# yl4579/StyleTTS2

Hardware: AMD Instinct MI355X
Metric: audio-seconds/sec (RTF^-1) end-to-end, 10 s utterance batch (higher is better)
Workload: dtype f32 (convs/linears: f16 hi/lo split, 3 MFMA products, fp32 accumulate)

## Files before the change

styletts2_amd/csrc/st2_misc.hip:

```cpp
#include "st2_common.h"

namespace {

__global__ __launch_bounds__(256) void conv1d_direct_kernel(const float* __restrict__ x, int64_t x_bs, int x_cs,
                                                            const float* __restrict__ w,
                                                            const float* __restrict__ bias, float* __restrict__ y,
                                                            int64_t y_bs, int y_cs, int C_in, int L_in_max, int L_out,
                                                            int ks, int stride, int pad, const int32_t* __restrict__ x_len,
                                                            const int32_t* __restrict__ y_len) {
  const int l = blockIdx.x * 256 + threadIdx.x;
  const int co = blockIdx.y;
  const int b = blockIdx.z;
  if (l >= L_out) return;
  const int L_in = x_len ? min(x_len[b], L_in_max) : L_in_max;
  if (y_len && l >= y_len[b]) {
    y[(int64_t)b * y_bs + (int64_t)co * y_cs + l] = 0.f;
    return;
  }
  const float* xb = x + (int64_t)b * x_bs;
  const float* wc = w + (int64_t)co * C_in * ks;
  float acc = 0.f;
  const int base = l * stride - pad;
  for (int ci = 0; ci < C_in; ++ci) {
    const float* xr = xb + (int64_t)ci * x_cs;
    for (int t = 0; t < ks; ++t) {
      const int p = base + t;
      if (p >= 0 && p < L_in) acc = fmaf(wc[ci * ks + t], xr[p], acc);
    }
  }
  if (bias) acc += bias[co];
  y[(int64_t)b * y_bs + (int64_t)co * y_cs + l] = acc;
}

__global__ __launch_bounds__(256) void phase_split_kernel(const float* __restrict__ x, int64_t x_bs, int x_cs, int L_in,
                                                          float* __restrict__ xp, int64_t p_bs, int p_cs, int Lu,
                                                          int stride, int pad) {
  const int pp = blockIdx.x * 256 + threadIdx.x;
  const int ci = blockIdx.y;
  const int b = blockIdx.z;
  if (pp >= Lu * stride) return;
  const int u = pp / stride;
  const int r = pp - u * stride;
  const int p = pp - pad;
  const float v = (p >= 0 && p < L_in) ? x[(int64_t)b * x_bs + (int64_t)ci * x_cs + p] : 0.f;
  xp[(int64_t)b * p_bs + (int64_t)(ci * stride + r) * p_cs + u] = v;
}

constexpr int CVT_TILE = 1024;
template <int S>
__global__ __launch_bounds__(256) void convt_interleave_kernel(const float* __restrict__ ph, int64_t p_bs, int p_cs,
                                                               const float* __restrict__ bias,
                                                               const float* __restrict__ add, int64_t a_bs, int a_cs,
                                                               float* __restrict__ out, int64_t o_bs, int o_cs, int C,
                                                               int stride_rt, int pad, int L_raw_max, int reflect_left,
                                                               float* __restrict__ part, int part_nt, int Lq_max,
                                                               const int32_t* __restrict__ q_len,
                                                               const int32_t* __restrict__ out_len) {
  extern __shared__ float cvt_tile[];
  __shared__ float red[2][4];
  const int stride = S ? S : stride_rt;
  const int co = blockIdx.y;
  const int b = blockIdx.z;
  const int L_out = out_len ? min(out_len[b], L_raw_max + reflect_left) : L_raw_max + reflect_left;
  const int Lq = q_len ? min(q_len[b], Lq_max) : Lq_max;
  const int o0 = blockIdx.x * CVT_TILE;
  if (o0 >= L_out) return;
  const int nq = CVT_TILE / stride + 3;
  const int nqp = nq | 1;
  const int l_lo = max(o0 - reflect_left, 0);
  const int q_lo = (l_lo + pad) / stride;
  {
    const float* pb = ph + (int64_t)b * p_bs + (int64_t)co * p_cs;
    const int total = stride * nq;
    constexpr int SB = 8;
    for (int e0 = threadIdx.x; e0 < total; e0 += 256 * SB) {
      float t[SB];
#pragma unroll
      for (int u = 0; u < SB; ++u) {
        const int e = min(e0 + u * 256, total - 1);
        const int r = e / nq, i = e - r * nq;
        t[u] = pb[(int64_t)r * C * p_cs + max(min(q_lo + i, Lq - 1), 0)];
      }
#pragma unroll
      for (int u = 0; u < SB; ++u) {
        const int e = e0 + u * 256;
        if (e < total) {
          const int r = e / nq, i = e - r * nq;
          cvt_tile[r * nqp + i] = (q_lo + i) < Lq ? t[u] : 0.f;
        }
      }
    }
  }
  __syncthreads();
  const float bj = bias ? bias[co] : 0.f;
  const float* ab = add ? add + (int64_t)b * a_bs + (int64_t)co * a_cs : nullptr;
  float* ob = out + (int64_t)b * o_bs + (int64_t)co * o_cs;
  auto staged_at = [&](int o) __attribute__((always_inline)) -> float {
    int l = o;
    if (reflect_left) l = (o == 0) ? 1 : o - 1;
    const int lp = l + pad;
    const int q = lp / stride;
    const int r = lp - q * stride;
    return cvt_tile[r * nqp + (q - q_lo)] + bj;
  };
  float shift = staged_at(o0);
  if (ab) shift += ab[o0];
  float s1 = 0.f, s2 = 0.f;
  const int o = o0 + 4 * threadIdx.x;
  if (o < L_out) {
    typedef float f4 __attribute__((ext_vector_type(4)));
    const bool full = o + 3 < L_out;
    const bool vec = full && ((reinterpret_cast<uintptr_t>(ob + o) & 15) == 0) && (!ab || (reinterpret_cast<uintptr_t>(ab + o) & 15) == 0);
    float v[4];
#pragma unroll
    for (int e = 0; e < 4; ++e) v[e] = (full || o + e < L_out) ? staged_at(o + e) : 0.f;
    if (ab) {
      if (vec) {
        const f4 a4 = *reinterpret_cast<const f4*>(ab + o);
#pragma unroll
        for (int e = 0; e < 4; ++e) v[e] += a4[e];
      } else {
#pragma unroll
        for (int e = 0; e < 4; ++e)
          if (full || o + e < L_out) v[e] += ab[o + e];
      }
    }
    if (vec) {
      *reinterpret_cast<f4*>(ob + o) = f4{v[0], v[1], v[2], v[3]};
    } else {
#pragma unroll
      for (int e = 0; e < 4; ++e)
        if (full || o + e < L_out) ob[o + e] = v[e];
    }
#pragma unroll
    for (int e = 0; e < 4; ++e)
      if (full || o + e < L_out) {
        const float dv = v[e] - shift;
        s1 += dv;
        s2 += dv * dv;
      }
  }
  if (part) {
    s1 = st2_wave_sum(s1);
    s2 = st2_wave_sum(s2);
    const int lane = threadIdx.x & 63, wave = threadIdx.x >> 6;
    if (lane == 0) {
      red[0][wave] = s1;
      red[1][wave] = s2;
    }
    __syncthreads();
    if (threadIdx.x == 0) {
      const float t1 = ((red[0][0] + red[0][1]) + red[0][2]) + red[0][3];
      const float t2 = ((red[1][0] + red[1][1]) + red[1][2]) + red[1][3];
      const int64_t slot = ((int64_t)b * C + co) * part_nt + blockIdx.x;
      reinterpret_cast<float2*>(part)[slot] = make_float2(t1, t2);
      part[(int64_t)gridDim.z * C * part_nt * 2 + slot] = shift;
    }
  }
}

__global__ __launch_bounds__(256) void adain_leaky_pool_kernel(const float* __restrict__ x, int64_t x_bs, int x_cs,
                                                               const float* __restrict__ stats,
                                                               const float* __restrict__ gamma,
                                                               const float* __restrict__ beta, int64_t gb_bs,
                                                               float slope, const float* __restrict__ w,
                                                               const float* __restrict__ bias, float* __restrict__ y,
                                                               int64_t y_bs, int y_cs, int C, int L_max,
                                                               const int32_t* __restrict__ len) {
  const int lo = blockIdx.x * 256 + threadIdx.x;
  const int c = blockIdx.y;
  const int b = blockIdx.z;
  const int L = len ? min(len[b], L_max) : L_max;
  if (lo >= 2 * L) return;
  const float mean = stats[((int64_t)b * C + c) * 2 + 0];
  const float rstd = stats[((int64_t)b * C + c) * 2 + 1];
  const float g = 1.0f + gamma[(int64_t)b * gb_bs + c];
  const float be = beta[(int64_t)b * gb_bs + c];
  const float* xr = x + (int64_t)b * x_bs + (int64_t)c * x_cs;
  auto act = [&](int i) -> float {
    float u = (xr[i] - mean) * rstd;
    u = g * u + be;
    return u >= 0.f ? u : u * slope;
  };
  const int j = lo >> 1;
  float v;
  if ((lo & 1) == 0) {
    v = act(j) * w[c * 3 + 1];
  } else {
    v = act(j) * w[c * 3 + 2];
    if (j + 1 < L) v += act(j + 1) * w[c * 3 + 0];
  }
  if (bias) v += bias[c];
  y[(int64_t)b * y_bs + (int64_t)c * y_cs + lo] = v;
}

__global__ __launch_bounds__(256) void add_chanvec_kernel(const float* __restrict__ x, int64_t x_bs, int x_cs,
                                                          const float* __restrict__ v, int64_t v_bs,
                                                          float* __restrict__ y, int64_t y_bs, int y_cs, int C,
                                                          int N) {
  const int n = blockIdx.x * 256 + threadIdx.x;
  const int c = blockIdx.y;
  const int b = blockIdx.z;
  if (n >= N) return;
  y[(int64_t)b * y_bs + (int64_t)c * y_cs + n] =
      x[(int64_t)b * x_bs + (int64_t)c * x_cs + n] + v[(int64_t)b * v_bs + c];
}

__global__ __launch_bounds__(64) void mean_tokens_kernel(const float* __restrict__ x, int64_t x_bs, int x_cs,
                                                         float* __restrict__ m, int64_t m_bs, int C, int N,
                                                         const int* __restrict__ len) {
  const int c = blockIdx.x;
  const int b = blockIdx.y;
  const float* xr = x + (int64_t)b * x_bs + (int64_t)c * x_cs;
  const int n_b = len ? min(max(len[b], 1), N) : N;
  double s = 0.0;
  for (int n = threadIdx.x; n < n_b; n += 64) s += (double)xr[n];
  s = st2_wave_sum(s);
  if (threadIdx.x == 0) m[(int64_t)b * m_bs + c] = (float)(s / (double)n_b);
}

__global__ __launch_bounds__(256) void axpbypcz_kernel(const float* __restrict__ x, float a,
                                                       const float* __restrict__ y, float b,
                                                       const float* __restrict__ z, float c, float* __restrict__ out,
                                                       int64_t n) {
  const int64_t i = (int64_t)blockIdx.x * 256 + threadIdx.x;
  if (i >= n) return;
  float v = a * x[i];
  if (y) v += b * y[i];
  if (z) v += c * z[i];
  out[i] = v;
}

}

extern "C" int st2_conv1d_direct(const float* x, int64_t x_bs, int32_t x_cs, const float* w, const float* bias,
                                 float* y, int64_t y_bs, int32_t y_cs, int32_t B, int32_t C_in, int32_t C_out,
                                 int32_t L_in, int32_t L_out, int32_t ks, int32_t stride, int32_t pad,
                                 void* stream) {
  return st2_conv1d_direct_len(x, x_bs, x_cs, w, bias, y, y_bs, y_cs, B, C_in, C_out, L_in, L_out, ks, stride, pad, nullptr,
                               nullptr, stream);
}

extern "C" int st2_conv1d_direct_len(const float* x, int64_t x_bs, int32_t x_cs, const float* w, const float* bias,
                                     float* y, int64_t y_bs, int32_t y_cs, int32_t B, int32_t C_in, int32_t C_out,
                                     int32_t L_in, int32_t L_out, int32_t ks, int32_t stride, int32_t pad,
                                     const int32_t* x_len, const int32_t* y_len, void* stream) {
  ST2_REQUIRE(x && w && y && B > 0 && C_in > 0 && C_out > 0 && L_in > 0 && L_out > 0 && ks > 0 && stride > 0,
              "st2_conv1d_direct: bad arguments");
  ST2_REQUIRE(C_out <= 65535 && B <= 65535, "st2_conv1d_direct: grid too large");
  hipStream_t s = reinterpret_cast<hipStream_t>(stream);
  hipLaunchKernelGGL(conv1d_direct_kernel, dim3(st2_cdiv(L_out, 256), C_out, B), dim3(256), 0, s, x, x_bs, x_cs, w,
                     bias, y, y_bs, y_cs, C_in, L_in, L_out, ks, stride, pad, x_len, y_len);
  ST2_CHECK_LAUNCH("st2_conv1d_direct");
  return 0;
}

extern "C" int st2_phase_split(const float* x, int64_t x_bs, int32_t x_cs, int32_t B, int32_t C, int32_t L_in,
                               int32_t stride, int32_t pad, float* xp, int64_t p_bs, int32_t p_cs, int32_t Lu,
                               void* stream) {
  ST2_REQUIRE(x && xp && B > 0 && C > 0 && L_in > 0 && stride > 0 && pad >= 0 && Lu > 0,
              "st2_phase_split: bad arguments");
  ST2_REQUIRE(C <= 65535 && B <= 65535 && (int64_t)Lu * stride < (int64_t)1 << 31, "st2_phase_split: grid too large");
  hipStream_t s = reinterpret_cast<hipStream_t>(stream);
  hipLaunchKernelGGL(phase_split_kernel, dim3(st2_cdiv((int64_t)Lu * stride, 256), C, B), dim3(256), 0, s, x, x_bs,
                     x_cs, L_in, xp, p_bs, p_cs, Lu, stride, pad);
  ST2_CHECK_LAUNCH("st2_phase_split");
  return 0;
}

extern "C" int st2_convt_interleave(const float* phases, int64_t p_bs, int32_t p_cs, int32_t Lq, const float* bias,
                                    const float* add, int64_t a_bs, int32_t a_cs, float* out, int64_t o_bs,
                                    int32_t o_cs, int32_t B, int32_t C, int32_t stride, int32_t pad, int32_t L_raw,
                                    int32_t reflect_left, void* stream) {
  return st2_convt_interleave_stats(phases, p_bs, p_cs, Lq, bias, add, a_bs, a_cs, out, o_bs, o_cs, B, C, stride, pad,
                                    L_raw, reflect_left, nullptr, 0, stream);
}

extern "C" int st2_convt_interleave_stats(const float* phases, int64_t p_bs, int32_t p_cs, int32_t Lq,
                                          const float* bias, const float* add, int64_t a_bs, int32_t a_cs, float* out,
                                          int64_t o_bs, int32_t o_cs, int32_t B, int32_t C, int32_t stride, int32_t pad,
                                          int32_t L_raw, int32_t reflect_left, float* part, int32_t part_nt,
                                          void* stream) {
  return st2_convt_interleave_stats_len(phases, p_bs, p_cs, Lq, bias, add, a_bs, a_cs, out, o_bs, o_cs, B, C, stride, pad, L_raw,
                                        reflect_left, part, part_nt, nullptr, nullptr, stream);
}

extern "C" int st2_convt_interleave_stats_len(const float* phases, int64_t p_bs, int32_t p_cs, int32_t Lq,
                                              const float* bias, const float* add, int64_t a_bs, int32_t a_cs, float* out,
                                              int64_t o_bs, int32_t o_cs, int32_t B, int32_t C, int32_t stride, int32_t pad,
                                              int32_t L_raw, int32_t reflect_left, float* part, int32_t part_nt,
                                              const int32_t* q_len, const int32_t* out_len, void* stream) {
  ST2_REQUIRE(!q_len == !out_len, "st2_convt_interleave_stats_len: q_len and out_len go together");
  ST2_REQUIRE(phases && out && B > 0 && C > 0 && stride > 0 && L_raw > 0 && Lq > 0,
              "st2_convt_interleave: bad arguments");
  ST2_REQUIRE(reflect_left == 0 || (reflect_left == 1 && L_raw >= 2), "st2_convt_interleave: bad reflect_left");
  ST2_REQUIRE(stride <= 64, "st2_convt_interleave: stride %d too large", stride);
  const int L_out = L_raw + reflect_left;
  const int nt = st2_cdiv(L_out, CVT_TILE);
  if (part) ST2_REQUIRE(part_nt >= nt && (reinterpret_cast<uintptr_t>(part) & 7) == 0,
                        "st2_convt_interleave: part_nt=%d < %d tiles (or part not 8-byte aligned)", part_nt, nt);
  ST2_REQUIRE(B <= 65535 && C <= 65535, "st2_convt_interleave: grid too large");
  hipStream_t s = reinterpret_cast<hipStream_t>(stream);
  const int nq = CVT_TILE / stride + 3;
  const size_t smem = (size_t)stride * (nq | 1) * sizeof(float);
#define ST2_CVT_LAUNCH(SV)                                                                                              \
  hipLaunchKernelGGL((convt_interleave_kernel<SV>), dim3(nt, C, B), dim3(256), smem, s, phases, p_bs, p_cs, bias, add, \
                     a_bs, a_cs, out, o_bs, o_cs, C, stride, pad, L_raw, reflect_left, part, part_nt, Lq, q_len, out_len)
  switch (stride) {
    case 2: ST2_CVT_LAUNCH(2); break;
    case 3: ST2_CVT_LAUNCH(3); break;
    case 5: ST2_CVT_LAUNCH(5); break;
    case 6: ST2_CVT_LAUNCH(6); break;
    case 10: ST2_CVT_LAUNCH(10); break;
    default: ST2_CVT_LAUNCH(0); break;
  }
#undef ST2_CVT_LAUNCH
  ST2_CHECK_LAUNCH("st2_convt_interleave");
  return 0;
}

extern "C" int st2_adain_leaky_pool(const float* x, int64_t x_bs, int32_t x_cs, const float* stats,
                                    const float* gamma, const float* beta, int64_t gb_bs, float slope, const float* w,
                                    const float* bias, float* y, int64_t y_bs, int32_t y_cs, int32_t B, int32_t C,
                                    int32_t L, void* stream) {
  return st2_adain_leaky_pool_len(x, x_bs, x_cs, stats, gamma, beta, gb_bs, slope, w, bias, y, y_bs, y_cs, B, C, L, nullptr,
                                  stream);
}

extern "C" int st2_adain_leaky_pool_len(const float* x, int64_t x_bs, int32_t x_cs, const float* stats,
                                        const float* gamma, const float* beta, int64_t gb_bs, float slope, const float* w,
                                        const float* bias, float* y, int64_t y_bs, int32_t y_cs, int32_t B, int32_t C,
                                        int32_t L, const int32_t* len, void* stream) {
  ST2_REQUIRE(x && stats && gamma && beta && w && y && B > 0 && C > 0 && L > 0,
              "st2_adain_leaky_pool: bad arguments");
  hipStream_t s = reinterpret_cast<hipStream_t>(stream);
  hipLaunchKernelGGL(adain_leaky_pool_kernel, dim3(st2_cdiv(2 * L, 256), C, B), dim3(256), 0, s, x, x_bs, x_cs,
                     stats, gamma, beta, gb_bs, slope, w, bias, y, y_bs, y_cs, C, L, len);
  ST2_CHECK_LAUNCH("st2_adain_leaky_pool");
  return 0;
}

extern "C" int st2_add_chanvec(const float* x, int64_t x_bs, int32_t x_cs, const float* v, int64_t v_bs, float* y,
                               int64_t y_bs, int32_t y_cs, int32_t B, int32_t C, int32_t N, void* stream) {
  ST2_REQUIRE(x && v && y && B > 0 && C > 0 && N > 0, "st2_add_chanvec: bad arguments");
  hipStream_t s = reinterpret_cast<hipStream_t>(stream);
  hipLaunchKernelGGL(add_chanvec_kernel, dim3(st2_cdiv(N, 256), C, B), dim3(256), 0, s, x, x_bs, x_cs, v, v_bs, y,
                     y_bs, y_cs, C, N);
  ST2_CHECK_LAUNCH("st2_add_chanvec");
  return 0;
}

extern "C" int st2_mean_tokens(const float* x, int64_t x_bs, int32_t x_cs, float* m, int64_t m_bs, int32_t B,
                               int32_t C, int32_t N, void* stream) {
  ST2_REQUIRE(x && m && B > 0 && C > 0 && N > 0, "st2_mean_tokens: bad arguments");
  hipStream_t s = reinterpret_cast<hipStream_t>(stream);
  hipLaunchKernelGGL(mean_tokens_kernel, dim3(C, B), dim3(64), 0, s, x, x_bs, x_cs, m, m_bs, C, N,
                     static_cast<const int*>(nullptr));
  ST2_CHECK_LAUNCH("st2_mean_tokens");
  return 0;
}

extern "C" int st2_mean_tokens_len(const float* x, int64_t x_bs, int32_t x_cs, float* m, int64_t m_bs, int32_t B,
                                   int32_t C, int32_t N, const int32_t* len, void* stream) {
  ST2_REQUIRE(x && m && B > 0 && C > 0 && N > 0, "st2_mean_tokens_len: bad arguments");
  hipStream_t s = reinterpret_cast<hipStream_t>(stream);
  hipLaunchKernelGGL(mean_tokens_kernel, dim3(C, B), dim3(64), 0, s, x, x_bs, x_cs, m, m_bs, C, N,
                     reinterpret_cast<const int*>(len));
  ST2_CHECK_LAUNCH("st2_mean_tokens_len");
  return 0;
}

extern "C" int st2_axpbypcz(const float* x, float a, const float* y, float b, const float* z, float c, float* out,
                            int64_t n, void* stream) {
  ST2_REQUIRE(x && out && n > 0, "st2_axpbypcz: bad arguments");
  hipStream_t s = reinterpret_cast<hipStream_t>(stream);
  hipLaunchKernelGGL(axpbypcz_kernel, dim3(st2_cdiv(n, 256)), dim3(256), 0, s, x, a, y, b, z, c, out, n);
  ST2_CHECK_LAUNCH("st2_axpbypcz");
  return 0;
}
```

styletts2_amd/csrc/st2_source.hip:

```cpp
#include "st2_common.h"

namespace {

__device__ __forceinline__ float torch_remainder1(float x) {
  float m = fmodf(x, 1.0f);
  if (m != 0.0f && m < 0.0f) m += 1.0f;
  return m;
}

__global__ __launch_bounds__(64) void sinegen_phase_kernel(const float* __restrict__ f0, int B, int F_max, int U, int H,
                                                           float sample_rate, float* __restrict__ phase_f,
                                                           const int32_t* __restrict__ f_len) {
  const int row = blockIdx.x;
  const int lane = threadIdx.x;
  const int b = row / H;
  const int h = row % H;
  const float mult = (float)(h + 1);
  const int F = f_len ? min(f_len[b], F_max) : F_max;
  const float* f = f0 + (int64_t)b * F_max;
  float* out = phase_f + ((int64_t)b * H + h) * F_max;
  const float two_pi_part = 3.14159274101257324219f;
  const float fu = (float)U;
  const int chunk = (F + 63) / 64;
  const int k0 = min(lane * chunk, F), k1 = min(k0 + chunk, F);
  double part = 0.0;
  for (int k = k0; k < k1; ++k) {
    const float fn = f[k] * mult;
    part += (double)torch_remainder1(fn / sample_rate);
  }
  double incl = part;
#pragma unroll
  for (int d = 1; d < 64; d <<= 1) {
    const double up = __shfl_up(incl, d, 64);
    if (lane >= d) incl += up;
  }
  double acc = __shfl_up(incl, 1, 64);
  if (lane == 0) acc = 0.0;
  for (int k = k0; k < k1; ++k) {
    const float fn = f[k] * mult;
    acc += (double)torch_remainder1(fn / sample_rate);
    const float c = (float)acc;
    out[k] = ((c * 2.0f) * two_pi_part) * fu;
  }
}

__global__ __launch_bounds__(256) void har_source_kernel(const float* __restrict__ f0, int F_max, int U, int H,
                                                         const float* __restrict__ noise,
                                                         const float* __restrict__ lin_w,
                                                         const float* __restrict__ lin_b, float sine_amp,
                                                         float noise_std, float voiced_threshold,
                                                         const float* __restrict__ phase_f,
                                                         float* __restrict__ out, const int32_t* __restrict__ f_len) {
  const int L_max = F_max * U;
  const int t = blockIdx.x * 256 + threadIdx.x;
  const int b = blockIdx.y;
  if (t >= L_max) return;
  const int F = f_len ? min(f_len[b], F_max) : F_max;
  const int L = F * U;
  if (t >= L) {
    out[(int64_t)b * L_max + t] = 0.f;
    return;
  }
  const float rs = (float)(1.0 / (double)U);
  float src = fmaf(rs, (float)t + 0.5f, -0.5f);
  src = src < 0.f ? 0.f : src;
  const int i0 = (int)src;
  const int i1 = min(i0 + 1, F - 1);
  const float w1 = src - (float)i0;
  const float w0 = 1.0f - w1;

  const float f0v = f0[(int64_t)b * F_max + t / U];
  const float uv = f0v > voiced_threshold ? 1.0f : 0.0f;
  const float noise_amp = uv * noise_std + ((1.0f - uv) * sine_amp) / 3.0f;

  const float* nz = noise + ((int64_t)b * L_max + t) * H;
  float acc = 0.f;
  for (int h = 0; h < H; ++h) {
    const float* pf = phase_f + ((int64_t)b * H + h) * F_max;
    const float ph = fmaf(w0, pf[i0], w1 * pf[i1]);
    const float sine = sinf(ph) * sine_amp;
    const float sw = sine * uv + noise_amp * nz[h];
    acc = fmaf(lin_w[h], sw, acc);
  }
  out[(int64_t)b * L_max + t] = tanhf(acc + lin_b[0]);
}

constexpr int MAXN = 32;
__global__ __launch_bounds__(256) void stft_kernel(const float* __restrict__ x, int L_max, int N, int hop,
                                                   float* __restrict__ har, int64_t har_bs, int har_cs,
                                                   const int32_t* __restrict__ len) {
  __shared__ float tw_c[MAXN], tw_s[MAXN], win[MAXN];
  if (threadIdx.x < N) {
    const double a = 2.0 * (double)threadIdx.x / (double)N;
    tw_c[threadIdx.x] = (float)cospi(a);
    tw_s[threadIdx.x] = (float)sinpi(a);
    win[threadIdx.x] = (float)(0.5 - 0.5 * cospi(a));
  }
  __syncthreads();
  const int m = blockIdx.x * 256 + threadIdx.x;
  const int b = blockIdx.y;
  if (m >= L_max / hop + 1) return;
  const int L = len ? min(max(len[b], N / 2 + 1), L_max) : L_max;
  const int M = L / hop + 1;
  const int NB = N / 2 + 1;
  float* hb = har + (int64_t)b * har_bs + m;
  if (m >= M) {
    for (int k = 0; k < 2 * NB; ++k) hb[(int64_t)k * har_cs] = 0.f;
    return;
  }
  const float* xb = x + (int64_t)b * L_max;
  float fr[MAXN];
  const int pad = N / 2;
#pragma unroll
  for (int n = 0; n < MAXN; ++n) {
    if (n < N) {
      int i = m * hop + n - pad;
      if (i < 0) i = -i;
      if (i >= L) i = 2 * (L - 1) - i;
      fr[n] = xb[i] * win[n];
    } else {
      fr[n] = 0.f;
    }
  }
  for (int k = 0; k < NB; ++k) {
    float re = 0.f, im = 0.f;
    int idx = 0;
#pragma unroll
    for (int n = 0; n < MAXN; ++n) {
      if (n < N) {
        re = fmaf(fr[n], tw_c[idx], re);
        im = fmaf(-fr[n], tw_s[idx], im);
        idx += k;
        if (idx >= N) idx -= N;
      }
    }
    hb[(int64_t)k * har_cs] = sqrtf(re * re + im * im);
    hb[(int64_t)(NB + k) * har_cs] = atan2f(im, re);
  }
}

__global__ __launch_bounds__(256) void istft_kernel(const float* __restrict__ sp, int64_t sp_bs, int sp_cs, int M_max,
                                                    int N, int hop, float* __restrict__ wave, int64_t wave_bs, int FRP,
                                                    const int32_t* __restrict__ m_len) {
  __shared__ float tw_c[MAXN], tw_s[MAXN], win[MAXN];
  extern __shared__ float ri[];
  if (threadIdx.x < N) {
    const double a = 2.0 * (double)threadIdx.x / (double)N;
    tw_c[threadIdx.x] = (float)cospi(a);
    tw_s[threadIdx.x] = (float)sinpi(a);
    win[threadIdx.x] = (float)(0.5 - 0.5 * cospi(a));
  }
  const int t = blockIdx.x * 256 + threadIdx.x;
  const int b = blockIdx.y;
  const int M = m_len ? min(max(m_len[b], 2), M_max) : M_max;
  const int Lw = hop * (M - 1);
  const int NB = N / 2 + 1;
  const float* sb = sp + (int64_t)b * sp_bs;
  {
    const int t0 = blockIdx.x * 256;
    const int tp0 = t0 + N / 2, tp1 = min(t0 + 255, Lw - 1) + N / 2;
    const int m_base = (tp0 - N + 1 <= 0) ? 0 : (tp0 - N + hop) / hop;
    const int m_last = min(tp1 / hop, M - 1);
    const int FR = m_last - m_base + 1;
    float* re_s = ri;
    float* im_s = ri + NB * FRP;
    for (int e = threadIdx.x; e < NB * FR; e += 256) {
      const int k = e / FR, f = e - k * FR;
      const float mag = sb[(int64_t)k * sp_cs + m_base + f];
      const float ph = sb[(int64_t)(NB + k) * sp_cs + m_base + f];
      re_s[k * FRP + f] = mag * cosf(ph);
      im_s[k * FRP + f] = mag * sinf(ph);
    }
  }
  __syncthreads();
  if (t >= Lw) {
    if (t < hop * (M_max - 1)) wave[(int64_t)b * wave_bs + t] = 0.f;
    return;
  }
  const int tp = t + N / 2;
  const int tp0 = (int)blockIdx.x * 256 + N / 2;
  const int m_base = (tp0 - N + 1 <= 0) ? 0 : (tp0 - N + hop) / hop;
  const float* re_s = ri;
  const float* im_s = ri + NB * FRP;
  int m_hi = tp / hop;
  if (m_hi > M - 1) m_hi = M - 1;
  int m_lo = (tp - N + hop) / hop;
  if (tp - N + 1 <= 0) m_lo = 0;
  const float inv_n = 1.0f / (float)N;
  float y = 0.f, env = 0.f;
  for (int m = m_lo; m <= m_hi; ++m) {
    const int n = tp - m * hop;
    float acc = 0.f;
    int idx = 0;
    const int f = m - m_base;
    for (int k = 0; k < NB; ++k) {
      const float re = re_s[k * FRP + f];
      const float im = im_s[k * FRP + f];
      if (k == 0 || k == N / 2) {
        acc += re * tw_c[idx];
      } else {
        acc += 2.0f * (re * tw_c[idx] - im * tw_s[idx]);
      }
      idx += n;
      if (idx >= N) idx -= N;
    }
    const float w = win[n];
    y += (acc * inv_n) * w;
    env += w * w;
  }
  wave[(int64_t)b * wave_bs + t] = y / env;
}

}

extern "C" int st2_har_source(const float* f0, int32_t B, int32_t F, int32_t U, int32_t H, const float* noise,
                              const float* lin_w, const float* lin_b, float sine_amp, float noise_std,
                              float voiced_threshold, float sample_rate, float* phase_scratch, float* out,
                              void* stream) {
  return st2_har_source_len(f0, B, F, U, H, noise, lin_w, lin_b, sine_amp, noise_std, voiced_threshold, sample_rate,
                            phase_scratch, out, nullptr, stream);
}

extern "C" int st2_har_source_len(const float* f0, int32_t B, int32_t F, int32_t U, int32_t H, const float* noise,
                                  const float* lin_w, const float* lin_b, float sine_amp, float noise_std,
                                  float voiced_threshold, float sample_rate, float* phase_scratch, float* out,
                                  const int32_t* f_len, void* stream) {
  ST2_REQUIRE(f0 && noise && lin_w && lin_b && phase_scratch && out, "st2_har_source: null pointer");
  ST2_REQUIRE(B > 0 && F > 0 && U > 0 && H > 0 && H <= 64, "st2_har_source: bad geometry");
  ST2_REQUIRE((int64_t)F * U < (1LL << 31), "st2_har_source: utterance too long");
  hipStream_t s = reinterpret_cast<hipStream_t>(stream);
  hipLaunchKernelGGL(sinegen_phase_kernel, dim3(B * H), dim3(64), 0, s, f0, B, F, U, H, sample_rate,
                     phase_scratch, f_len);
  ST2_CHECK_LAUNCH("st2_har_source(phase)");
  hipLaunchKernelGGL(har_source_kernel, dim3(st2_cdiv((int64_t)F * U, 256), B), dim3(256), 0, s, f0, F, U, H, noise,
                     lin_w, lin_b, sine_amp, noise_std, voiced_threshold, phase_scratch, out, f_len);
  ST2_CHECK_LAUNCH("st2_har_source");
  return 0;
}

extern "C" int st2_stft_mag_phase(const float* x, int32_t B, int32_t L, int32_t n_fft, int32_t hop, float* har,
                                  int64_t har_bs, int32_t har_cs, void* stream) {
  return st2_stft_mag_phase_len(x, B, L, n_fft, hop, har, har_bs, har_cs, nullptr, stream);
}

extern "C" int st2_stft_mag_phase_len(const float* x, int32_t B, int32_t L, int32_t n_fft, int32_t hop, float* har,
                                      int64_t har_bs, int32_t har_cs, const int32_t* len, void* stream) {
  ST2_REQUIRE(x && har && B > 0 && L > 0, "st2_stft_mag_phase: bad arguments");
  ST2_REQUIRE(n_fft >= 2 && n_fft <= MAXN && (n_fft % 2) == 0 && hop > 0 && L > n_fft / 2,
              "st2_stft_mag_phase: n_fft=%d hop=%d L=%d unsupported", n_fft, hop, L);
  hipStream_t s = reinterpret_cast<hipStream_t>(stream);
  const int M = L / hop + 1;
  hipLaunchKernelGGL(stft_kernel, dim3(st2_cdiv(M, 256), B), dim3(256), 0, s, x, L, n_fft, hop, har, har_bs, har_cs, len);
  ST2_CHECK_LAUNCH("st2_stft_mag_phase");
  return 0;
}

extern "C" int st2_istft(const float* sp, int64_t sp_bs, int32_t sp_cs, int32_t B, int32_t M, int32_t n_fft,
                         int32_t hop, float* wave, int64_t wave_bs, void* stream) {
  return st2_istft_len(sp, sp_bs, sp_cs, B, M, n_fft, hop, wave, wave_bs, nullptr, stream);
}

extern "C" int st2_istft_len(const float* sp, int64_t sp_bs, int32_t sp_cs, int32_t B, int32_t M, int32_t n_fft,
                             int32_t hop, float* wave, int64_t wave_bs, const int32_t* m_len, void* stream) {
  ST2_REQUIRE(sp && wave && B > 0 && M > 1, "st2_istft: bad arguments");
  ST2_REQUIRE(n_fft >= 2 && n_fft <= MAXN && (n_fft % 2) == 0 && hop > 0 && (n_fft % hop) == 0,
              "st2_istft: n_fft=%d hop=%d unsupported", n_fft, hop);
  hipStream_t s = reinterpret_cast<hipStream_t>(stream);
  const int Lw = hop * (M - 1);
  const int FRP = (256 / hop + n_fft / hop + 3) | 1;
  const size_t smem = (size_t)2 * (n_fft / 2 + 1) * FRP * sizeof(float);
  hipLaunchKernelGGL(istft_kernel, dim3(st2_cdiv(Lw, 256), B), dim3(256), smem, s, sp, sp_bs, sp_cs, M, n_fft, hop, wave,
                     wave_bs, FRP, m_len);
  ST2_CHECK_LAUNCH("st2_istft");
  return 0;
}
```

Baseline: 4978.

## Specialize STFT/iSTFT for n_fft=20 hop=5 and vectorize AdaIN-leaky-pool

Adds a template STFT kernel for n_fft=20, hop=5 that stages the reflect-padded input window in shared memory and fully unrolls the DFT with compile-time twiddle indices. Adds a dedicated iSTFT kernel that computes each frame's inverse DFT once into a shared-memory tile and then overlap-adds from it. The AdaIN+leaky+transposed-pool kernel now handles two input samples per thread, using float2 loads and float4 stores. These target redundant global loads and per-output recomputation in the vocoder's STFT/iSTFT and upsampling steps, at the cost of more specialized code paths and shared-memory use.

```diff
diff --git a/styletts2_amd/csrc/st2_misc.hip b/styletts2_amd/csrc/st2_misc.hip
--- a/styletts2_amd/csrc/st2_misc.hip
+++ b/styletts2_amd/csrc/st2_misc.hip
@@ -167,31 +167,62 @@
                                                                const float* __restrict__ bias, float* __restrict__ y,
                                                                int64_t y_bs, int y_cs, int C, int L_max,
                                                                const int32_t* __restrict__ len) {
-  const int lo = blockIdx.x * 256 + threadIdx.x;
+  const int j0 = 2 * (blockIdx.x * 256 + threadIdx.x);
   const int c = blockIdx.y;
   const int b = blockIdx.z;
   const int L = len ? min(len[b], L_max) : L_max;
-  if (lo >= 2 * L) return;
+  if (j0 >= L) return;
   const float mean = stats[((int64_t)b * C + c) * 2 + 0];
   const float rstd = stats[((int64_t)b * C + c) * 2 + 1];
   const float g = 1.0f + gamma[(int64_t)b * gb_bs + c];
   const float be = beta[(int64_t)b * gb_bs + c];
   const float* xr = x + (int64_t)b * x_bs + (int64_t)c * x_cs;
-  auto act = [&](int i) -> float {
-    float u = (xr[i] - mean) * rstd;
+  float* yr = y + (int64_t)b * y_bs + (int64_t)c * y_cs + 2 * (int64_t)j0;
+  auto act = [&](float xv) -> float {
+    float u = (xv - mean) * rstd;
     u = g * u + be;
     return u >= 0.f ? u : u * slope;
   };
-  const int j = lo >> 1;
-  float v;
-  if ((lo & 1) == 0) {
-    v = act(j) * w[c * 3 + 1];
+  const float w0 = w[c * 3 + 0], w1 = w[c * 3 + 1], w2 = w[c * 3 + 2];
+  const bool two = j0 + 1 < L;
+  float x0, x1 = 0.f;
+  if (two && (reinterpret_cast<uintptr_t>(xr + j0) & 7) == 0) {
+    const float2 x2 = *reinterpret_cast<const float2*>(xr + j0);
+    x0 = x2.x;
+    x1 = x2.y;
   } else {
-    v = act(j) * w[c * 3 + 2];
-    if (j + 1 < L) v += act(j + 1) * w[c * 3 + 0];
-  }
-  if (bias) v += bias[c];
-  y[(int64_t)b * y_bs + (int64_t)c * y_cs + lo] = v;
+    x0 = xr[j0];
+    if (two) x1 = xr[j0 + 1];
+  }
+  const float a0 = act(x0);
+  float v0 = a0 * w1;
+  float v1 = a0 * w2;
+  float v2 = 0.f, v3 = 0.f;
+  if (two) {
+    const float a1 = act(x1);
+    v1 += a1 * w0;
+    v2 = a1 * w1;
+    v3 = a1 * w2;
+    if (j0 + 2 < L) v3 += act(xr[j0 + 2]) * w0;
+  }
+  if (bias) {
+    const float bc = bias[c];
+    v0 += bc;
+    v1 += bc;
+    v2 += bc;
+    v3 += bc;
+  }
+  if (two && (reinterpret_cast<uintptr_t>(yr) & 15) == 0) {
+    typedef float f4 __attribute__((ext_vector_type(4)));
+    *reinterpret_cast<f4*>(yr) = f4{v0, v1, v2, v3};
+  } else {
+    yr[0] = v0;
+    yr[1] = v1;
+    if (two) {
+      yr[2] = v2;
+      yr[3] = v3;
+    }
+  }
 }
 
 __global__ __launch_bounds__(256) void add_chanvec_kernel(const float* __restrict__ x, int64_t x_bs, int x_cs,
@@ -334,7 +365,7 @@
   ST2_REQUIRE(x && stats && gamma && beta && w && y && B > 0 && C > 0 && L > 0,
               "st2_adain_leaky_pool: bad arguments");
   hipStream_t s = reinterpret_cast<hipStream_t>(stream);
-  hipLaunchKernelGGL(adain_leaky_pool_kernel, dim3(st2_cdiv(2 * L, 256), C, B), dim3(256), 0, s, x, x_bs, x_cs,
+  hipLaunchKernelGGL(adain_leaky_pool_kernel, dim3(st2_cdiv(L, 512), C, B), dim3(256), 0, s, x, x_bs, x_cs,
                      stats, gamma, beta, gb_bs, slope, w, bias, y, y_bs, y_cs, C, L, len);
   ST2_CHECK_LAUNCH("st2_adain_leaky_pool");
   return 0;
diff --git a/styletts2_amd/csrc/st2_source.hip b/styletts2_amd/csrc/st2_source.hip
--- a/styletts2_amd/csrc/st2_source.hip
+++ b/styletts2_amd/csrc/st2_source.hip
@@ -86,56 +86,94 @@
 }
 
 constexpr int MAXN = 32;
-__global__ __launch_bounds__(256) void stft_kernel(const float* __restrict__ x, int L_max, int N, int hop,
+template <int NT, int HOP>
+__global__ __launch_bounds__(256) void stft_kernel(const float* __restrict__ x, int L_max, int N_rt, int hop_rt,
                                                    float* __restrict__ har, int64_t har_bs, int har_cs,
                                                    const int32_t* __restrict__ len) {
   __shared__ float tw_c[MAXN], tw_s[MAXN], win[MAXN];
+  __shared__ float xs_s[NT ? 256 * HOP + NT : 1];
+  const int N = NT ? NT : N_rt;
+  const int hop = NT ? HOP : hop_rt;
   if (threadIdx.x < N) {
     const double a = 2.0 * (double)threadIdx.x / (double)N;
     tw_c[threadIdx.x] = (float)cospi(a);
     tw_s[threadIdx.x] = (float)sinpi(a);
     win[threadIdx.x] = (float)(0.5 - 0.5 * cospi(a));
   }
-  __syncthreads();
   const int m = blockIdx.x * 256 + threadIdx.x;
   const int b = blockIdx.y;
-  if (m >= L_max / hop + 1) return;
   const int L = len ? min(max(len[b], N / 2 + 1), L_max) : L_max;
   const int M = L / hop + 1;
+  const int pad = N / 2;
+  const float* xb = x + (int64_t)b * L_max;
+  if (NT) {
+    const int i_base = blockIdx.x * 256 * hop - pad;
+    const int j_end = min(256 * hop + N, (M - 1) * hop + N - (i_base + pad));
+    for (int j = threadIdx.x; j < j_end; j += 256) {
+      int i = i_base + j;
+      if (i < 0) i = -i;
+      if (i >= L) i = 2 * (L - 1) - i;
+      xs_s[j] = xb[i];
+    }
+  }
+  __syncthreads();
+  if (m >= L_max / hop + 1) return;
   const int NB = N / 2 + 1;
   float* hb = har + (int64_t)b * har_bs + m;
   if (m >= M) {
     for (int k = 0; k < 2 * NB; ++k) hb[(int64_t)k * har_cs] = 0.f;
     return;
   }
-  const float* xb = x + (int64_t)b * L_max;
   float fr[MAXN];
-  const int pad = N / 2;
 #pragma unroll
   for (int n = 0; n < MAXN; ++n) {
     if (n < N) {
-      int i = m * hop + n - pad;
-      if (i < 0) i = -i;
-      if (i >= L) i = 2 * (L - 1) - i;
-      fr[n] = xb[i] * win[n];
+      if (NT) {
+        fr[n] = xs_s[threadIdx.x * hop + n] * win[n];
+      } else {
+        int i = m * hop + n - pad;
+        if (i < 0) i = -i;
+        if (i >= L) i = 2 * (L - 1) - i;
+        fr[n] = xb[i] * win[n];
+      }
     } else {
       fr[n] = 0.f;
     }
   }
-  for (int k = 0; k < NB; ++k) {
-    float re = 0.f, im = 0.f;
-    int idx = 0;
-#pragma unroll
-    for (int n = 0; n < MAXN; ++n) {
-      if (n < N) {
-        re = fmaf(fr[n], tw_c[idx], re);
-        im = fmaf(-fr[n], tw_s[idx], im);
-        idx += k;
-        if (idx >= N) idx -= N;
-      }
-    }
-    hb[(int64_t)k * har_cs] = sqrtf(re * re + im * im);
-    hb[(int64_t)(NB + k) * har_cs] = atan2f(im, re);
+  if constexpr (NT != 0) {
+    float cr[NT], sr[NT];
+#pragma unroll
+    for (int n = 0; n < NT; ++n) {
+      cr[n] = tw_c[n];
+      sr[n] = tw_s[n];
+    }
+#pragma unroll
+    for (int k = 0; k < NT / 2 + 1; ++k) {
+      float re = 0.f, im = 0.f;
+#pragma unroll
+      for (int n = 0; n < NT; ++n) {
+        re = fmaf(fr[n], cr[(n * k) % NT], re);
+        im = fmaf(-fr[n], sr[(n * k) % NT], im);
+      }
+      hb[(int64_t)k * har_cs] = sqrtf(re * re + im * im);
+      hb[(int64_t)(NB + k) * har_cs] = atan2f(im, re);
+    }
+  } else {
+    for (int k = 0; k < NB; ++k) {
+      float re = 0.f, im = 0.f;
+      int idx = 0;
+#pragma unroll
+      for (int n = 0; n < MAXN; ++n) {
+        if (n < N) {
+          re = fmaf(fr[n], tw_c[idx], re);
+          im = fmaf(-fr[n], tw_s[idx], im);
+          idx += k;
+          if (idx >= N) idx -= N;
+        }
+      }
+      hb[(int64_t)k * har_cs] = sqrtf(re * re + im * im);
+      hb[(int64_t)(NB + k) * har_cs] = atan2f(im, re);
+    }
   }
 }
 
@@ -211,6 +249,97 @@
   wave[(int64_t)b * wave_bs + t] = y / env;
 }
 
+constexpr int I20_N = 20, I20_HOP = 5, I20_NB = 11;
+constexpr int I20_TILE = 1260;
+constexpr int I20_FR = I20_TILE / I20_HOP + 3;
+constexpr int I20_P = 269;
+static_assert(I20_FR <= 256 && I20_FR <= I20_P && I20_TILE % I20_HOP == 0, "istft20 tile");
+__global__ __launch_bounds__(256) void istft20_kernel(const float* __restrict__ sp, int64_t sp_bs, int sp_cs, int M_max,
+                                                      float* __restrict__ wave, int64_t wave_bs,
+                                                      const int32_t* __restrict__ m_len) {
+  constexpr int N = I20_N, hop = I20_HOP, NB = I20_NB;
+  __shared__ float tw_c[N], tw_s[N], win[N];
+  __shared__ float ft[N * I20_P];
+  const int b = blockIdx.y;
+  const int t0 = blockIdx.x * I20_TILE;
+  const int M = m_len ? min(max(m_len[b], 2), M_max) : M_max;
+  const int Lw = hop * (M - 1);
+  float* wb = wave + (int64_t)b * wave_bs;
+  if (t0 >= Lw) {
+    for (int o = threadIdx.x; o < I20_TILE; o += 256)
+      if (t0 + o < hop * (M_max - 1)) wb[t0 + o] = 0.f;
+    return;
+  }
+  if (threadIdx.x < N) {
+    const double a = 2.0 * (double)threadIdx.x / (double)N;
+    tw_c[threadIdx.x] = (float)cospi(a);
+    tw_s[threadIdx.x] = (float)sinpi(a);
+    win[threadIdx.x] = (float)(0.5 - 0.5 * cospi(a));
+  }
+  __syncthreads();
+  const int m_base = t0 == 0 ? 0 : t0 / hop - 1;
+  {
+    const int m = m_base + (int)threadIdx.x;
+    if ((int)threadIdx.x < I20_FR && m <= M - 1) {
+      const float* sb = sp + (int64_t)b * sp_bs + m;
+      float mag[NB], ph[NB], re[NB], im[NB];
+#pragma unroll
+      for (int k = 0; k < NB; ++k) {
+        mag[k] = sb[(int64_t)k * sp_cs];
+        ph[k] = sb[(int64_t)(NB + k) * sp_cs];
+      }
+#pragma unroll
+      for (int k = 0; k < NB; ++k) {
+        re[k] = mag[k] * cosf(ph[k]);
+        im[k] = mag[k] * sinf(ph[k]);
+      }
+      float cr[N], sr[N], wr[N];
+#pragma unroll
+      for (int n = 0; n < N; ++n) {
+        cr[n] = tw_c[n];
+        sr[n] = tw_s[n];
+        wr[n] = win[n];
+      }
+      const float inv_n = 1.0f / (float)N;
+#pragma unroll
+      for (int n = 0; n < N; ++n) {
+        float acc = 0.f;
+#pragma unroll
+        for (int k = 0; k < NB; ++k) {
+          const int idx = (n * k) % N;
+          if (k == 0 || k == N / 2) {
+            acc += re[k] * cr[idx];
+          } else {
+            acc += 2.0f * (re[k] * cr[idx] - im[k] * sr[idx]);
+          }
+        }
+        ft[n * I20_P + threadIdx.x] = (acc * inv_n) * wr[n];
+      }
+    }
+  }
+  __syncthreads();
+  for (int o = threadIdx.x; o < I20_TILE; o += 256) {
+    const int t = t0 + o;
+    if (t >= Lw) {
+      if (t < hop * (M_max - 1)) wb[t] = 0.f;
+      continue;
+    }
+    const int tp = t + N / 2;
+    int m_hi = tp / hop;
+    if (m_hi > M - 1) m_hi = M - 1;
+    int m_lo = (tp - N + hop) / hop;
+    if (tp - N + 1 <= 0) m_lo = 0;
+    float y = 0.f, env = 0.f;
+    for (int m = m_lo; m <= m_hi; ++m) {
+      const int n = tp - m * hop;
+      const float w = win[n];
+      y += ft[n * I20_P + (m - m_base)];
+      env += w * w;
+    }
+    wb[t] = y / env;
+  }
+}
+
 }
 
 extern "C" int st2_har_source(const float* f0, int32_t B, int32_t F, int32_t U, int32_t H, const float* noise,
@@ -250,7 +379,12 @@
               "st2_stft_mag_phase: n_fft=%d hop=%d L=%d unsupported", n_fft, hop, L);
   hipStream_t s = reinterpret_cast<hipStream_t>(stream);
   const int M = L / hop + 1;
-  hipLaunchKernelGGL(stft_kernel, dim3(st2_cdiv(M, 256), B), dim3(256), 0, s, x, L, n_fft, hop, har, har_bs, har_cs, len);
+  if (n_fft == 20 && hop == 5)
+    hipLaunchKernelGGL((stft_kernel<20, 5>), dim3(st2_cdiv(M, 256), B), dim3(256), 0, s, x, L, n_fft, hop, har, har_bs, har_cs,
+                       len);
+  else
+    hipLaunchKernelGGL((stft_kernel<0, 0>), dim3(st2_cdiv(M, 256), B), dim3(256), 0, s, x, L, n_fft, hop, har, har_bs, har_cs,
+                       len);
   ST2_CHECK_LAUNCH("st2_stft_mag_phase");
   return 0;
 }
@@ -267,6 +401,12 @@
               "st2_istft: n_fft=%d hop=%d unsupported", n_fft, hop);
   hipStream_t s = reinterpret_cast<hipStream_t>(stream);
   const int Lw = hop * (M - 1);
+  if (n_fft == I20_N && hop == I20_HOP) {
+    hipLaunchKernelGGL(istft20_kernel, dim3(st2_cdiv(Lw, I20_TILE), B), dim3(256), 0, s, sp, sp_bs, sp_cs, M, wave, wave_bs,
+                       m_len);
+    ST2_CHECK_LAUNCH("st2_istft");
+    return 0;
+  }
   const int FRP = (256 / hop + n_fft / hop + 3) | 1;
   const size_t smem = (size_t)2 * (n_fft / 2 + 1) * FRP * sizeof(float);
   hipLaunchKernelGGL(istft_kernel, dim3(st2_cdiv(Lw, 256), B), dim3(256), smem, s, sp, sp_bs, sp_cs, M, n_fft, hop, wave,
```

After: 4996 (median of 6 runs). Within noise of the previous version (+0.4%).
